# Griffan/VerifyBamID

Hardware: AMD Instinct MI355X
Metric: llk_evals_per_sec (higher is better)
Workload: dtype f64; 1 GPU; synthetic pileup 100000 markers x depth 30, --NumPC 4 (BASELINE.json configs[2] shape); parallelism=1 GPU, rccl_world_size=1, launched_by=single process, reads=2999230, active_markers=100000, distinct_codes=42, device=gfx950:sramecc+:xnack-

## Files before the change

### verifybamid_amd/csrc/kernel_debug.h

```cpp
#ifndef VB2_KERNEL_DEBUG_H_
#define VB2_KERNEL_DEBUG_H_

#ifndef VB2_ABLATE
#define VB2_ABLATE 0
#endif
#ifndef VB2_FLAG_RELEASE
#define VB2_FLAG_RELEASE 1
#endif
#ifndef VB2_SOFT_PROLOGUE
#define VB2_SOFT_PROLOGUE 1
#endif
#ifndef VB2_CTRL_PRIO
#define VB2_CTRL_PRIO 3
#endif
#ifndef VB2_STAMP_ROUND
#define VB2_STAMP_ROUND 0
#endif

namespace vb2 {
constexpr int kAblNoMap = 1, kAblNoTable = 2, kAblNoItems = 4, kAblNoReads = 8, kAblNoEpi = 16, kAblNoSignal = 32, kAblNoMul = 64, kAblNoRowLoads = 128;
constexpr int kAblate = VB2_ABLATE;
}

#ifdef VB2_WITH_STAMPS
#define VB2_STAMPS_OF(L) ((L).stamps)
#else
#define VB2_STAMPS_OF(L) (static_cast<unsigned long long*>(nullptr))
#endif

#ifdef VB2_ITEM_PROF
#define VB2_IP_T(var) const unsigned long long var = __builtin_readcyclecounter()
#define VB2_IP_USE(x) asm volatile("" ::"v"(x))
#else
#define VB2_IP_T(var)
#define VB2_IP_USE(x)
#endif

#endif
```

### verifybamid_amd/csrc/llk_kernels.hip

```cpp
#include "llk_kernels.h"

#include <hip/hip_runtime.h>
#include <link.h>

#include "kernel_debug.h"
#include "tile_sched.h"
#include "tunables.h"
#ifndef VB2_SIMD_DEAL
#define VB2_SIMD_DEAL 1
#endif

#include <algorithm>
#include <atomic>
#include <cstring>
#include <type_traits>
#include <vector>

namespace vb2 {

__device__ __forceinline__ void pair_of(int p, int& g1, int& g2)
{
    g1 = p >> 1;
    const int lo = p & 1;
    g2 = lo + (lo >= g1 ? 1 : 0);
// ... 212 lines not shown
    const double val = (alpha * e1 + one_minus_alpha * e2) * p_err +
                       (alpha * n1 + one_minus_alpha * n2) * p_ok;
    return log_tab(val, ltab_addr);
}

__device__ __forceinline__ double prob_entry(double alpha, double p_err, int g1, int g2)
{
    const double p_ok = 1.0 - p_err;
    const double e1 = (double)g1 * (1.0 / 6.0), e2 = (double)g2 * (1.0 / 6.0);
    const double n1 = 1.0 - 0.5 * (double)g1, n2 = 1.0 - 0.5 * (double)g2;
    const double one_minus_alpha = 1.0 - alpha;
    double val = (alpha * e1 + one_minus_alpha * e2) * p_err +
                 (alpha * n1 + one_minus_alpha * n2) * p_ok;
    return val >= 0.0 ? val : __builtin_nan("");
}

__device__ __forceinline__ void initial_gf(double af, double* gf)
{
    af = vmin_f64(vmax_f64(af, 0.00005), 0.99995);
    gf[0] = (1 - af) * (1 - af);
    gf[1] = 2 * (af) * (1 - af);
    gf[2] = af * af;
}


constexpr int kExpTabDoubles = 64 * 32;
constexpr int kPrefetch = 8;
constexpr int kPrefetchL2 = 2;

__device__ __forceinline__ void lane_map(int lane, int& m, int& g)
{
    const int q = (lane >> 2) & 7;
    const int nib = (0x76452310u >> (4 * q)) & 7;
    g = (nib & 1) + 2 * (lane >> 5);
    m = ((nib >> 1) << 2) + (lane & 3);
}
__device__ __forceinline__ int lane_of(int m, int g)
{
    const int idx = ((g & 1) << 2) + (m >> 2);
    const int q = (0x74216530u >> (4 * idx)) & 7;
    return ((g >> 1) << 5) + (q << 2) + (m & 3);
}

__device__ __forceinline__ int lane_xchg_i32(int x, int off, int partner)
{
    if (off == 1) return __builtin_amdgcn_update_dpp(0, x, 0xB1, 0xf, 0xf, true);
    if (off == 2) return __builtin_amdgcn_update_dpp(0, x, 0x4E, 0xf, 0xf, true);
    if (off == 4) {
        const int a = __builtin_amdgcn_update_dpp(0, x, 0x124, 0xf, 0x5, false);
        return __builtin_amdgcn_update_dpp(a, x, 0x12C, 0xf, 0xa, false);
    }
    return __shfl(x, partner, 64);
}
__device__ __forceinline__ double lane_xchg_f64(double x, int off, int partner)
{
    if (off == 1 || off == 2 || off == 4)
        return __hiloint2double(lane_xchg_i32(__double2hiint(x), off, partner), lane_xchg_i32(__double2loint(x), off, partner));
    return __shfl(x, partner, 64);
}

template <int MODE> struct Geom { static constexpr int kMaxWaves = 16, kBlocksPerCU = 1, kWavesPerSimd = 4; };
template <int MODE> struct ModeNp { static constexpr int value = MODE == 2 ? 8 : MODE == 4 ? 1 : MODE == 5 ? 2 : 4; };

struct InlinePoints {
    int count;
    double v[kInlinePointDoubles];
};

struct NoHook {
    __device__ bool on_block() const { return false; }
    __device__ bool mine() const { return false; }
    __device__ void run() {}
    __device__ bool keep_etab() const { return false; }
    __device__ bool prim_in_lds() const { return false; }
    __device__ bool keep_prim() const { return false; }
    __device__ double* sum_stage() const { return nullptr; }
    __device__ uint32_t cache_rec() const { return 0u; }
    __device__ unsigned int* sync_word() const { return nullptr; }
    __device__ bool collect_only() const { return false; }
    __device__ bool no_collect() const { return false; }
};
__host__ __device__ __forceinline__ bool eval_is_dynamic(const DeviceLayout& L, uint32_t nblk, int nwave, int ngrp)
{
    const uint32_t max_tiles_blk = owned_most(L.pd ? 1 : 0, (uint32_t)L.num_mt, nblk);
    return max_tiles_blk * (uint32_t)ngrp <= (uint32_t)(L.dyn_limit * nwave);
}

template <int MODE, bool W16 = false, class Hook = NoHook, bool STREAM = false, int QUEUE = -1, int KSEL = 0,
          bool LCACHE = false, int ESH = 8, bool PD = false, int SPLIT = 0>
__device__ __forceinline__ void
eval_body(const DeviceLayout& L, const double* ip_v, const int ip_count, const double* __restrict__ points, int num_valid,
          double* __restrict__ partials, double* __restrict__ llk_out,
          unsigned int* __restrict__ ticket, unsigned long long* __restrict__ done_flag,
          unsigned long long done_seq, const uint32_t blk, const uint32_t nblk,
          unsigned int* __restrict__ batch_done, unsigned int batch_active, const int ngrp_in,
          const unsigned long long tag, const Schedule sch, const bool coherent_points = false,
          const int tid_in = -1, const double* lds_rows = nullptr ,
          Hook hook = Hook())
{
    extern __shared__ __attribute__((aligned(16))) double lds[];
    static_assert(MODE >= 2 && MODE <= 5, "wave shapes 2..5");
    static_assert(!PD || ESH == 8, "probability-domain contexts have no exp table");
    static_assert(!(PD && W16) || ((MODE == 4 || MODE == 5) && STREAM), "8-bit step lists: cohort steps of one and two points");
    static_assert(!SPLIT || (PD && MODE == 2 && QUEUE == 1 && !STREAM && !LCACHE), "split launches: the 8-point shape on the queue");
    constexpr int OSH = PD ? 1 : 0;
    constexpr bool ONEGRP = MODE != 2 || STREAM;
    constexpr int KAF = KSEL > 0 ? 0 : -1;
    constexpr int BTL = MODE == 4 ? 1 : 2;
    constexpr int TPW = MODE == 3 ? 2 : (MODE == 4 || MODE == 5) ? 4 : 1;
    constexpr int SLOTS = 4 / TPW;
    constexpr int NP = SLOTS * BTL;
    const int row_bytes = MODE == 2 ? kRowBytesWide : L.row_bytes;
    const int RS = row_bytes >> 3;
    const int nrow = L.num_code + 1;
    const int nthread = blockDim.x;
    const int nwave = nthread >> 6;
    const int k = KSEL > 0 ? KSEL : L.num_pc;
    const int stride = 2 * k + 1;
    constexpr int NVS = SPLIT ? SPLIT : 1;
    const int g_per = SPLIT ? (ngrp_in + NVS - 1) / NVS : ngrp_in;
    const int g_lo = SPLIT ? (int)(blk % (uint32_t)NVS) * g_per : 0;
    const int ngrp = ONEGRP ? 1 : SPLIT ? (ngrp_in - g_lo < g_per ? ngrp_in - g_lo : g_per) : ngrp_in;
    const int p_off = g_lo * NP;
    const uint32_t vstep = SPLIT ? nblk / (uint32_t)NVS : 0u, vb0 = SPLIT ? blk / (uint32_t)NVS : blk;
    const double* const known_af_p = KAF == 0 ? nullptr : L.known_af;
    const int NPT = NP * ngrp;
    constexpr int kEtabCopies = (1 << ESH) / 8, kEtabDoubles = PD ? 0 : 64 * kEtabCopies;
    constexpr int kLtabDoubles = PD ? 0 : kLogTabDoubles;
    double* etab = lds;
    double* ltab = lds + kEtabDoubles;
    double* tab = ltab + kLtabDoubles;
    double* red = tab + ngrp * nrow * RS;
    unsigned int* queue = reinterpret_cast<unsigned int*>(red + NVS * NPT);
    double* pts = red + NVS * NPT + 2;
    double* ptq = pts + (size_t)NPT * stride + ((NPT * stride) & 1);
    const size_t prim_off = (size_t)(ptq - lds) + (size_t)NPT * 2 * k;
    double2* prim_lds = reinterpret_cast<double2*>(lds + prim_off + (prim_off & 1));
    double* tile_llk = reinterpret_cast<double*>(prim_lds + L.num_prim);

    const int tid = tid_in >= 0 ? tid_in : (int)threadIdx.x;
    const int lane = tid & 63;
    const int wave = __builtin_amdgcn_readfirstlane(tid >> 6);
    int m, g4;
    lane_map(lane, m, g4);
    const int g = g4 & (SLOTS - 1);
    const int half = TPW == 1 ? 0 : g4 / SLOTS;
    const bool stamp_this = VB2_STAMP_ROUND == 0 || (unsigned)(tag & 0xffffffffull) == (unsigned)VB2_STAMP_ROUND;
#ifdef VB2_ITEM_PROF
    unsigned long long* stamps = nullptr;
#else
    unsigned long long* stamps = (VB2_STAMPS_OF(L) && stamp_this) ? VB2_STAMPS_OF(L) + (size_t)blk * 8 : nullptr;
#endif
    if (stamps && tid == 0) { stamps[0] = wall_clock64(); stamps[4] = 0; }

    const bool collect_only = hook.collect_only();
    if (collect_only && hook.mine()) hook.run();
    if (!collect_only) {
    const bool hook_blk = hook.on_block(), hook_mine = hook.mine();
    unsigned int* const soft_word = PD ? hook.sync_word() : nullptr;
    const bool soft = hook_blk && soft_word != nullptr;
    if (soft && hook_mine) hook.run();
    const int ptid = !soft ? tid : hook_mine ? 0x3fffffff : tid - 64, pnthread = soft ? nthread - 64 : nthread;
    unsigned int soft_gen = 0;
    auto prologue_sync = [&]() {
        if (!soft) { __syncthreads(); return; }
        if (hook_mine) return;
        soft_gen += (unsigned int)(nwave - 1);
        if (lane == 0) __hip_atomic_fetch_add(soft_word, 1u, __ATOMIC_RELAXED, __HIP_MEMORY_SCOPE_WORKGROUP);
        while (__hip_atomic_load(soft_word, __ATOMIC_RELAXED, __HIP_MEMORY_SCOPE_WORKGROUP) < soft_gen) __builtin_amdgcn_s_sleep(1);
        asm volatile("" ::: "memory");
    };
    if (ptid == 0) *queue = (unsigned int)(nwave - (hook_blk ? 1 : 0));
    for (int e = ptid; e < NPT * stride; e += pnthread) {
        const int b = e / stride;
        const int src = p_off + b < num_valid ? p_off + b : num_valid - 1;
        const int idx = src * stride + (e - b * stride);
        const double v = (kAblate & kAblNoMap) ? 0.01 * (double)(1 + idx % 7)
                         : lds_rows ? lds_rows[idx]
                         : ip_count > 0 ? ip_v[idx]
                         : coherent_points ? __hip_atomic_load(&points[idx], __ATOMIC_RELAXED, __HIP_MEMORY_SCOPE_AGENT)
                                           : points[idx];
        pts[e] = v;
        const int c = e - b * stride;
        if (c < 2 * k) ptq[((b / BTL) * 2 * k + c) * BTL + (b % BTL)] = v;
    }
    if (!PD && !hook.keep_etab() && tid < kLogTabDoubles / 2)
        reinterpret_cast<double2*>(ltab)[tid] = kLogTabRows[tid];
    if (!PD && !hook.keep_etab())
        for (int jb = 2 * wave; jb < 64; jb += 2 * nwave) {
            const double t0 = kExp2Tab[jb], t1 = kExp2Tab[jb + 1];
            const double tv = lane < 32 ? exp_tab_entry(t0, jb) : exp_tab_entry(t1, jb + 1);
            if constexpr (ESH == 8) etab[jb * 32 + lane] = tv;
            else if ((lane & 31) < kEtabCopies) etab[(jb + (lane >> 5)) * kEtabCopies + (lane & 31)] = tv;
        }
    const bool prim_kept = hook.prim_in_lds() && hook.keep_prim();
    const bool staged = ngrp > 1 || (hook.prim_in_lds() && !prim_kept) || (PD && L.num_pair > 0 && !prim_kept);
    if (staged)
        for (int e = ptid; e < L.num_prim; e += pnthread) prim_lds[e] = L.prim[e];
    const bool early_table = lds_rows != nullptr && !staged;
    if (!early_table) prologue_sync();
    if (stamps && (soft ? ptid : tid) == 0) stamps[1] = wall_clock64();

    const uint32_t ltab_addr = lds_byte_addr(ltab);
    const int num_single = PD ? L.num_prim - L.num_pair : L.num_prim;
    for (int e = ptid; e < ((kAblate & kAblNoTable) ? 0 : num_single * 6 * NP); e += pnthread) {
        const int pi = e / (6 * NP);
        const int bp = e - pi * (6 * NP);
        const int bb = bp / 6, p = bp - bb * 6;
        const double2 rec = (staged || prim_kept) ? prim_lds[pi] : L.prim[pi];
        const uint32_t pr = (uint32_t)__double_as_longlong(rec.y);
        const int dc = (int)(pr & 0xffffu), twin = (int)(pr >> 16);
        int g1, g2;
        pair_of(p, g1, g2);
        if constexpr (PD && !ONEGRP) {
            constexpr int kSide = 3;
            for (int g0 = 0; g0 < ngrp; g0 += kSide) {
                double v3[kSide], r3[kSide];
                double* cell3[kSide];
#pragma unroll
                for (int u = 0; u < kSide; ++u) {
                    const int ge = g0 + u < ngrp ? g0 + u : ngrp - 1;
                    v3[u] = prob_entry(pts[(ge * NP + bb) * stride + 2 * k], rec.x, g1, g2);
                    r3[u] = v3[u];
                    cell3[u] = tab + (size_t)ge * nrow * RS + dc * RS + bp;
                    *cell3[u] = r3[u];
                }
                const int kq = twin & 0xff, pstride = RS * (int)(int8_t)(twin >> 8);
                for (int n = 1; n < kq; ++n) {
#pragma unroll
                    for (int u = 0; u < kSide; ++u) {
                        r3[u] *= v3[u];
                        cell3[u] += pstride;
                        *cell3[u] = r3[u];
                    }
                }
            }
        } else
#pragma clang loop unroll(disable)
        for (int grp_e = 0; grp_e < ngrp; ++grp_e) {
            const double alpha_e = early_table ? lds_rows[(bb < num_valid ? bb : num_valid - 1) * stride + 2 * k]
                                               : pts[(grp_e * NP + bb) * stride + 2 * k];
            double* gtab = tab + (size_t)grp_e * nrow * RS;
            if constexpr (PD) {
                const double v = prob_entry(alpha_e, rec.x, g1, g2);
                double r = v;
                double* cell = gtab + dc * RS + bp;
                constexpr int kMir = kPdAltOffset / 8;
                const int mir = kMir + bb * 6 + (5 - p) - bp;
                *cell = r;
                if constexpr (NP <= 4 && STREAM) cell[mir] = r;
                const int kq = twin & 0xff, pstride = RS * (int)(int8_t)(twin >> 8);
                for (int n = 1; n < kq; ++n) {
                    r *= v;
                    cell += pstride;
                    *cell = r;
                    if constexpr (NP <= 4 && STREAM) cell[mir] = r;
                }
            } else {
                const double v = table_entry(alpha_e, rec.x, g1, g2, ltab_addr);
                const double tv = W16 ? 0.5 * v : v;
                gtab[dc * RS + bp] = tv;
                if (twin != 0xffff) gtab[twin * RS + bb * 6 + (5 - p)] = tv;
            }
        }
    }
    for (int e = ptid; e < ngrp * RS; e += pnthread) {
        const int grp_e = e / RS;
        tab[((size_t)grp_e * nrow + L.num_code) * RS + (e - grp_e * RS)] = PD ? 1.0 : 0.0;
    }
    if constexpr (PD) {
        for (int level = 0; level < 2 && L.num_pair > 0 && !(kAblate & kAblNoTable); ++level) {
            const int nrec = level == 0 ? L.num_pair - L.num_pair2 : L.num_pair2;
            if (nrec == 0) break;
            prologue_sync();
            const double2* const prec = prim_lds + num_single + (level == 0 ? 0 : L.num_pair - L.num_pair2);
            for (int e = ptid; e < nrec * 6 * NP; e += pnthread) {
                const int pi = e / (6 * NP);
                const int bp = e - pi * (6 * NP);
                const double2 rec = prec[pi];
                const uint32_t ab = (uint32_t)__double_as_longlong(rec.x), dst = (uint32_t)__double_as_longlong(rec.y);
                const int ra = (int)(ab & 0xffffu) * RS + bp, rb = (int)(ab >> 16) * RS + bp, rd = (int)dst * RS + bp;
                constexpr int kMir = kPdAltOffset / 8;
                const int bb = bp / 6, p = bp - bb * 6;
                const int mir = kMir + bb * 6 + (5 - p) - bp;
#pragma clang loop unroll(disable)
                for (int grp_e = 0; grp_e < ngrp; ++grp_e) {
                    double* gtab = tab + (size_t)grp_e * nrow * RS;
                    const double v = gtab[ra] * gtab[rb];
                    gtab[rd] = v;
                    if constexpr (NP <= 4 && STREAM) gtab[rd + mir] = v;
                }
            }
        }
    }
    prologue_sync();
    if (stamps && (soft ? ptid : tid) == 0) stamps[2] = wall_clock64();

    const uint32_t nt_v0 = owned_count(OSH, (uint32_t)L.num_mt, vb0, nblk);
    const uint32_t nt_v1 = SPLIT ? owned_count(OSH, (uint32_t)L.num_mt, vb0 + vstep, nblk) : 0u;
    const uint32_t nt_v2 = SPLIT > 2 ? owned_count(OSH, (uint32_t)L.num_mt, vb0 + 2u * vstep, nblk) : 0u;
    auto nt_of = [&](uint32_t vs) { return vs == 0u ? nt_v0 : vs == 1u ? nt_v1 : nt_v2; };
    const uint32_t ntile_blk = nt_v0;
    const size_t mp = L.m_pad;
    const uint32_t nunit = SPLIT ? (uint32_t)NVS * ntile_blk : (ntile_blk + TPW - 1) / TPW;
    const uint32_t nitem = (kAblate & kAblNoItems) ? 0u : nunit * (uint32_t)ngrp;
    const float inv_nunit = 1.0f / (float)(nunit ? nunit : 1u);
    const uint32_t ngrp_magic = ngrp > 1 ? 0xFFFFFFFFu / (uint32_t)ngrp + 1u : 0u;
    const bool dyn = QUEUE < 0 ? eval_is_dynamic(L, nblk, nwave, ngrp) : QUEUE != 0;
    typedef unsigned int __attribute__((ext_vector_type(2))) vuint2;
    typedef __attribute__((address_space(1))) const vuint2 g_cuint2;
    typedef __attribute__((address_space(1))) const double g_cdouble;
    typedef __attribute__((address_space(1))) const char g_cchar;
    g_cuint2* const g_rec = (g_cuint2*)(W16 ? L.mt_rec16 : L.mt_rec);
    g_cuint2* const g_codes = (g_cuint2*)(W16 ? L.codes16 : L.codes);
    typedef __attribute__((address_space(1))) const uint32_t g_cuint;
    typedef __attribute__((address_space(3))) const uint32_t lds_cuint;
    typedef typename std::conditional<PD, uint32_t, vuint2>::type RowWord;
    constexpr uint32_t kRowBytes = PD ? kMtMarkers * 4u : kMtMarkers * 8u, kLaneBytes = PD ? 4u : 8u;
    g_cdouble* const g_ediag = (g_cdouble*)L.ediag;
    g_cdouble* const g_ud = (g_cdouble*)L.ud;
    g_cdouble* const g_mu = (g_cdouble*)L.mu;
    g_cdouble* const g_kaf = (g_cdouble*)known_af_p;
    auto tile_product = [&](ScaledProd* p, bool cross) {
#pragma unroll
        for (int off = 8; off >= 1; off >>= 1) {
            const int partner = lane_of(m ^ off, g4);
#pragma unroll
            for (int t = 0; t < BTL; ++t) {
                p[t].m *= lane_xchg_f64(p[t].m, off, partner);
                p[t].e += lane_xchg_f64(p[t].e, off, partner);
            }
        }
        if (!cross) return;
#pragma unroll
        for (int off = SLOTS; off < 4; off <<= 1) {
            const int partner = lane_of(m, g4 ^ off);
#pragma unroll
            for (int t = 0; t < BTL; ++t) {
                p[t].m *= __shfl(p[t].m, partner, 64);
                p[t].e += __shfl(p[t].e, partner, 64);
            }
        }
    };
    LaneProd wave_prod[BTL];
#pragma unroll
    for (int t = 0; t < BTL; ++t) wave_prod[t] = LaneProd{1.0, 0};
    int nfactor = 0;
    auto renorm_wave = [&]() {
#pragma unroll
        for (int t = 0; t < BTL; ++t) {
            wave_prod[t].e += __builtin_amdgcn_frexp_exp(wave_prod[t].m);
            wave_prod[t].m = __builtin_amdgcn_frexp_mant(wave_prod[t].m);
        }
        nfactor = 0;
    };
    uint32_t grp_wave = 0;
    auto flush_wave = [&](uint32_t grp) {
// ... 445 lines not shown
                if (r < end && (r & 1)) row_step(kS1, alt_tag, alt_tag, kNotFirst);
                while (r + 1 < end) {
                    row_step(kS0, alt_tag, alt_tag, kNotFirst);
                    row_step(kS1, alt_tag, alt_tag, kNotFirst);
                }
                if (r < end) row_step(kS0, alt_tag, alt_tag, kNotFirst);
            };
            rows_of_kind(rows_ra, kRef);
            if ((steps_ref & 1) && r == rows_ra && r < rows) {
                if (r & 1) row_step(kS1, kRef, kAltT, kNotFirst);
                else row_step(kS0, kRef, kAltT, kNotFirst);
            }
            rows_of_kind(rows, kAltT);
            if constexpr (PIPE) {
                issue_rows(rec_n2, have_next);
                cst_nx = other_const(mt_next, have_next);
                rec_nx = rec_n2;
            }
        } else if constexpr (PIPE) {
            const bool more = __any(rows > kPf);
            walk_block(0, more, std::false_type());
            if (more)
                for (int s0 = kPf; s0 < rows; s0 += kPf) walk_block(s0, true, std::false_type());
            issue_rows(rec_n2, have_next);
            cst_nx = other_const(mt_next, have_next);
            rec_nx = rec_n2;
        } else if constexpr (PEEL) {
            if (rows > 0) {
                walk_block(0, true, std::true_type());
                for (int s0 = kPf; s0 < rows; s0 += kPf) walk_block(s0, true, std::false_type());
            } else {
#pragma unroll
                for (int i = 0; i < BTL * 6; ++i) acc[i] = cst;
            }
        } else {
            for (int s0 = 0; s0 < rows; s0 += kPf) walk_block(s0, true, std::false_type());
        }

        __builtin_amdgcn_s_setprio(0);
#ifdef VB2_STAMP_CTRL
        if (stamps && lane == 0 && wave == 1 && !hook_blk) stamps[3] = wall_clock64();
#else
        if (stamps && lane == 0 && wave == 1) stamps[3] = wall_clock64();
#endif
        VB2_IP_USE(acc[0]); VB2_IP_USE(acc[BTL * 6 - 1]);
        VB2_IP_T(ip_t3);
        VB2_IP_USE(e0); VB2_IP_USE(e1); VB2_IP_USE(e2); VB2_IP_USE(mur); VB2_IP_USE(udr[0]); VB2_IP_USE(udr[3]);
        VB2_IP_T(ip_t4);
        double lk_m[BTL];
        int lk_e[BTL];
        marker_lk(live, pos, acc, e0, e1, e2, udr, mur, my_ptq, lk_m, lk_e, cst);
        VB2_IP_USE(lk_m[0]); VB2_IP_USE(lk_m[BTL - 1]);
        VB2_IP_T(ip_t5);
        if (!dyn) {
#pragma unroll
            for (int t = 0; t < BTL; ++t) {
                wave_prod[t].m *= lk_m[t];
                wave_prod[t].e += lk_e[t];
            }
            if (++nfactor == kLazyRenorm) renorm_wave();
            if (have_sched) {
                ++s_i;
                idx = PIPE ? idx_next : (s_i < s_end ? (uint32_t)sch.item[s_i] : nitem);
                continue;
            }
            ++round;
            idx = round * (uint32_t)nwave + ((round & 1u) ? (uint32_t)(nwave - 1 - wave) : (uint32_t)wave);
            continue;
        }
#pragma unroll
        for (int off = 8; off >= 1; off >>= 1) {
            const int partner = lane_of(m ^ off, g4);
#pragma unroll
            for (int t = 0; t < BTL; ++t) {
                lk_m[t] *= lane_xchg_f64(lk_m[t], off, partner);
                lk_e[t] += lane_xchg_i32(lk_e[t], off, partner);
            }
        }
        if (m == 0 && have_tile) {
#pragma unroll
            for (int t = 0; t < BTL; ++t) {
                const size_t o = ((((size_t)grp * NVS + vs) * ntile_blk + it) * NP + g * BTL + t) * 2;
                tile_llk[o] = lk_m[t];
                tile_llk[o + 1] = (double)lk_e[t];
            }
        }
        VB2_IP_T(ip_t6);
        idx = draw_item();
#ifdef VB2_ITEM_PROF
        {
            const unsigned long long ip_t7 = __builtin_readcyclecounter();
            ip_sum[0] += ip_t1 - ip_t0; ip_sum[1] += ip_t2 - ip_t1; ip_sum[2] += ip_t3 - ip_t2; ip_sum[3] += ip_t4 - ip_t3;
            ip_sum[4] += ip_t5 - ip_t4; ip_sum[5] += ip_t6 - ip_t5; ip_sum[6] += ip_t7 - ip_t6; ip_sum[7] += 1;
        }
#endif
    }
#ifdef VB2_ITEM_PROF
    if (VB2_STAMPS_OF(L) && lane == 0 && dyn)
        for (int i = 0; i < 8; ++i) atomicAdd(&VB2_STAMPS_OF(L)[(size_t)blk * 8 + i], ip_sum[i]);
#endif
    if (!dyn) {
        for (uint32_t grp = grp_wave; grp < (uint32_t)ngrp; ++grp) flush_wave(grp);
    }

    if (stamps && lane == 0 && !hook_mine) atomicMax(&stamps[4], wall_clock64());
    const uint32_t nres = dyn ? ntile_blk : (uint32_t)nwave;
    __syncthreads();
    {
        const uint32_t j16 = (uint32_t)lane & 15u;
        for (int b = tid >> 4; b < NVS * NPT; b += nthread >> 4) {
            const int vsb = SPLIT ? b / NPT : 0, bl = b - vsb * NPT;
            const int grp = bl / NP, bb = bl - grp * NP;
            ScaledProd p{1.0, 0.0};
            const uint32_t nres_b = SPLIT ? nt_of((uint32_t)vsb) : nres;
            for (uint32_t i = j16; i < nres_b; i += 16) {
                const size_t o = ((((size_t)grp * NVS + vsb) * nres + i) * NP + bb) * 2;
                p.m *= tile_llk[o];
                p.e += tile_llk[o + 1];
                sp_renorm(p);
            }
            auto row_move = [&](double x, auto ctrl) -> double {
                constexpr int kCtrl = decltype(ctrl)::value;
                return __hiloint2double(__builtin_amdgcn_update_dpp(0, __double2hiint(x), kCtrl, 0xf, 0xf, false),
                                        __builtin_amdgcn_update_dpp(0, __double2loint(x), kCtrl, 0xf, 0xf, false));
            };
            auto row_step = [&](auto ctrl) {
                const double om = row_move(p.m, ctrl), oe = row_move(p.e, ctrl);
                p.m *= om;
                p.e += oe;
            };
            row_step(std::integral_constant<int, 0x140>());
            row_step(std::integral_constant<int, 0x141>());
            row_step(std::integral_constant<int, 0xB1>());
            row_step(std::integral_constant<int, 0x4E>());
            sp_renorm(p);
            if (j16 == 0) red[b] = log_nonneg(p.m) + p.e * 6.93147180559945286227e-01;
        }
    }
    __syncthreads();
    if (VB2_STAMPS_OF(L) && tid == 0) {
        const unsigned long long t5 = wall_clock64();
        if (stamps) stamps[5] = t5;
        if (blk == 0 && nblk > 32 && !hook.no_collect()) VB2_STAMPS_OF(L)[20 * 8 + 7] += t5 - VB2_STAMPS_OF(L)[7];
    }
    }
    auto put_result = [&](int b, double v) {
        if (done_flag) __hip_atomic_store(&llk_out[b], v, __ATOMIC_RELAXED, __HIP_MEMORY_SCOPE_SYSTEM);
        else llk_out[b] = v;
    };
    if (ticket == nullptr) {
        if (tid < NPT) partials[(size_t)tid * nblk + blk] = red[tid];
        return;
    }
    if (tag == 0) {
        if (tid < NVS * NPT) {
            const int vsb = SPLIT ? tid / NPT : 0, bl = tid - vsb * NPT;
            __hip_atomic_store(&partials[(size_t)(p_off + bl) * nblk + (vb0 + (uint32_t)vsb * vstep)], red[tid],
                               __ATOMIC_RELAXED, __HIP_MEMORY_SCOPE_AGENT);
        }
        asm volatile("s_waitcnt vmcnt(0)" ::: "memory");
        __syncthreads();
        unsigned int* last_flag = queue;
        if (tid == 0) {
            const unsigned int t = __hip_atomic_fetch_add(ticket, 1u, __ATOMIC_RELAXED,
                                                          __HIP_MEMORY_SCOPE_AGENT);
            *last_flag = (t == nblk - 1) ? 1u : 0u;
        }
        __syncthreads();
        if (*last_flag == 0u) return;
        const int nbt = (int)nblk;
        constexpr int kSide = 3;
        for (int b0 = wave; b0 < num_valid; b0 += kSide * nwave) {
            double s[kSide];
#pragma unroll
            for (int u = 0; u < kSide; ++u) s[u] = 0;
            for (int base = 0; base < nbt; base += 8 * 64) {
                double x[kSide][8];
#pragma unroll
                for (int u = 0; u < kSide; ++u) {
                    const int b = b0 + u * nwave;
                    const double* p = partials + (size_t)(b < num_valid ? b : b0) * nbt;
#pragma unroll
                    for (int q = 0; q < 8; ++q) {
                        const int i = base + q * 64 + lane;
                        x[u][q] = i < nbt ? __hip_atomic_load(&p[i], __ATOMIC_RELAXED, __HIP_MEMORY_SCOPE_AGENT)
                                          : 0.0;
                    }
                }
#pragma unroll
                for (int u = 0; u < kSide; ++u)
#pragma unroll
                    for (int q = 0; q < 8; ++q) s[u] += x[u][q];
            }
#pragma unroll
            for (int u = 0; u < kSide; ++u) {
                const int b = b0 + u * nwave;
                const double t = wave_sum(s[u]);
                if (lane == 0 && b < num_valid) put_result(b, t);
            }
        }
        if (tid == 0) __hip_atomic_store(ticket, 0u, __ATOMIC_RELAXED, __HIP_MEMORY_SCOPE_AGENT);
    } else {
    unsigned long long* pw = reinterpret_cast<unsigned long long*>(partials);
    if (wave == 0 && !collect_only) {
        const unsigned long long bits = lane < NPT ? (unsigned long long)__double_as_longlong(red[lane]) : 0ull;
        if (lane < NPT)
            __hip_atomic_store(&pw[(size_t)lane * nblk + blk], bits, __ATOMIC_RELAXED, __HIP_MEMORY_SCOPE_AGENT);
        unsigned long long x = lane < NPT ? word_hash(bits, (unsigned)lane) : 0ull;
        int top = 1;
        while (top < NPT) top <<= 1;
        for (int off = top >> 1; off >= 1; off >>= 1) x ^= __shfl_xor(x, off, 64);
        if (lane == 0)
            __hip_atomic_store(&pw[(size_t)NPT * nblk + blk], x ^ resident_mix(tag), __ATOMIC_RELAXED,
                               __HIP_MEMORY_SCOPE_AGENT);
    }
    if (collect_only ? false : (blk != 0 || hook.no_collect())) return;
    if (!hook.sum_stage()) __syncthreads();
    const int nb = (int)nblk;
    double* stage = hook.sum_stage() ? hook.sum_stage() : lds;
    {
        const unsigned long long want = resident_mix(tag);
        const unsigned long long t_wait = wall_clock64();
        for (int b = tid; b < nb; b += nthread) {
            for (unsigned it = 0;; ++it) {
                unsigned long long x = __hip_atomic_load(&pw[(size_t)NPT * nb + b], __ATOMIC_RELAXED,
                                                         __HIP_MEMORY_SCOPE_AGENT);
                for (int w0 = 0; w0 < NPT; w0 += NP) {
                    unsigned long long v[NP];
#pragma unroll
                    for (int u = 0; u < NP; ++u)
                        v[u] = __hip_atomic_load(&pw[(size_t)(w0 + u) * nb + b], __ATOMIC_RELAXED,
                                                 __HIP_MEMORY_SCOPE_AGENT);
#pragma unroll
                    for (int u = 0; u < NP; ++u) {
                        x ^= word_hash(v[u], (unsigned)(w0 + u));
                        stage[(size_t)(w0 + u) * nb + b] = __longlong_as_double((long long)v[u]);
                    }
                }
                if (x == want) break;
                if ((it & 63) == 63 && wall_clock64() - t_wait > kHandoffGiveUpTicks) {
                    for (int w = 0; w < NPT; ++w) stage[(size_t)w * nb + b] = __builtin_nan("");
                    break;
                }
                __builtin_amdgcn_s_sleep(1);
            }
        }
    }
    __syncthreads();
    for (int b = wave; b < num_valid; b += nwave) {
        const double* p = stage + (size_t)b * nb;
        double s = 0;
        for (int base = 0; base < nb; base += 8 * 64) {
            double x[8];
#pragma unroll
            for (int q = 0; q < 8; ++q) {
                const int i = base + q * 64 + lane;
                x[q] = i < nb ? p[i] : 0.0;
            }
#pragma unroll
            for (int q = 0; q < 8; ++q) s += x[q];
        }
        s = wave_sum(s);
        if (lane == 0) put_result(b, s);
    }
    }
    if (VB2_STAMPS_OF(L) && tid == 0) {
        const unsigned long long t6 = wall_clock64();
        if (stamps) stamps[6] = t6;
        if ((collect_only || (blk == 0 && !hook.no_collect())) && nblk > 32) VB2_STAMPS_OF(L)[21 * 8 + 7] += t6 - VB2_STAMPS_OF(L)[7];
    }
    if (done_flag && !(kAblate & kAblNoSignal)) {
        asm volatile("s_waitcnt vmcnt(0)" ::: "memory");
        __syncthreads();
        if (tid == 0) {
            bool signal = true;
            if (batch_done) {
                const unsigned int t = __hip_atomic_fetch_add(batch_done, 1u, __ATOMIC_RELAXED, __HIP_MEMORY_SCOPE_AGENT);
                signal = (t == batch_active - 1);
                if (signal) __hip_atomic_store(batch_done, 0u, __ATOMIC_RELAXED, __HIP_MEMORY_SCOPE_AGENT);
            }
            if (signal)
                __hip_atomic_store(done_flag, done_seq, VB2_FLAG_RELEASE ? __ATOMIC_RELEASE : __ATOMIC_RELAXED, __HIP_MEMORY_SCOPE_SYSTEM);
        }
    }
}

template <int MODE, int QUEUE, int KSEL = 0, bool PD = false>
__global__ void __launch_bounds__(Geom<MODE>::kMaxWaves * 64, Geom<MODE>::kWavesPerSimd)
llk_eval_kernel(const DeviceLayout L, const InlinePoints ip, const double* __restrict__ points,
                int num_valid, double* __restrict__ partials, double* __restrict__ llk_out,
                unsigned int* __restrict__ ticket, unsigned long long* __restrict__ done_flag,
                unsigned long long done_seq, int ngrp, unsigned long long tag, const Schedule sch)
{
    eval_body<MODE, false, NoHook, false, QUEUE, KSEL, false, 8, PD>(L, ip.v, ip.count, points, num_valid, partials, llk_out, ticket,
                                                                     done_flag, done_seq, blockIdx.x, gridDim.x, nullptr, 0u, ngrp, tag, sch);
}

template <int KSEL, int S>
__global__ void __launch_bounds__(Geom<2>::kMaxWaves * 64, Geom<2>::kWavesPerSimd)
llk_eval_split_kernel(const DeviceLayout L, const double* __restrict__ points, int num_valid, double* __restrict__ partials,
                      double* __restrict__ llk_out, unsigned int* __restrict__ ticket, unsigned long long* __restrict__ done_flag,
                      unsigned long long done_seq, int ngrp)
{
    eval_body<2, false, NoHook, false, 1, KSEL, false, 8, true, S>(L, nullptr, 0, points, num_valid, partials, llk_out, ticket, done_flag,
                                                                     done_seq, blockIdx.x, gridDim.x, nullptr, 0u, ngrp, 0ull,
                                                                     Schedule{nullptr, nullptr});
}

template <int KSEL, bool PD = false>
__global__ void __launch_bounds__(Geom<2>::kMaxWaves * 64, Geom<2>::kWavesPerSimd)
llk_eval_passes_kernel(const DeviceLayout L, const double* __restrict__ points, int num_valid, int points_per_pass,
                       double* __restrict__ partials, double* __restrict__ llk_out, unsigned int* __restrict__ tickets,
                       unsigned long long* __restrict__ done_flag, unsigned long long done_seq,
                       unsigned long long* __restrict__ scratch_flag)
{
    const int stride = 2 * L.num_pc + 1;
    int pass = 0;
    for (int first = 0; first < num_valid; first += points_per_pass, ++pass) {
        const int left = num_valid - first;
        const int nv = left < points_per_pass ? left : points_per_pass;
        const bool last = left <= points_per_pass;
        if (pass > 0) __syncthreads();
        eval_body<2, false, NoHook, false, 1, KSEL, false, (PD ? 8 : 6), PD>(
            L, nullptr, 0, points + (size_t)first * stride, nv, partials + (size_t)first * gridDim.x, llk_out + first,
            tickets + pass, (last || !done_flag) ? done_flag : scratch_flag, done_seq, blockIdx.x, gridDim.x, nullptr, 0u,
            (nv + 7) / 8, 0ull, Schedule{nullptr, nullptr});
    }
}

#define VB2_PASSES_KERNEL_ARGS                                                                                           \
    const DeviceLayout, const double*, int, int, double*, double*, unsigned int*, unsigned long long*, unsigned long long, \
        unsigned long long*
#if defined(VB2_TU_MAIN)
extern template __global__ void llk_eval_passes_kernel<4>(VB2_PASSES_KERNEL_ARGS);
extern template __global__ void llk_eval_passes_kernel<2>(VB2_PASSES_KERNEL_ARGS);
extern template __global__ void llk_eval_passes_kernel<0>(VB2_PASSES_KERNEL_ARGS);
extern template __global__ void llk_eval_passes_kernel<4, true>(VB2_PASSES_KERNEL_ARGS);
extern template __global__ void llk_eval_passes_kernel<2, true>(VB2_PASSES_KERNEL_ARGS);
extern template __global__ void llk_eval_passes_kernel<0, true>(VB2_PASSES_KERNEL_ARGS);
#elif defined(VB2_TU_PASSES)
template __global__ void llk_eval_passes_kernel<4>(VB2_PASSES_KERNEL_ARGS);
template __global__ void llk_eval_passes_kernel<2>(VB2_PASSES_KERNEL_ARGS);
template __global__ void llk_eval_passes_kernel<0>(VB2_PASSES_KERNEL_ARGS);
template __global__ void llk_eval_passes_kernel<4, true>(VB2_PASSES_KERNEL_ARGS);
template __global__ void llk_eval_passes_kernel<2, true>(VB2_PASSES_KERNEL_ARGS);
template __global__ void llk_eval_passes_kernel<0, true>(VB2_PASSES_KERNEL_ARGS);
#endif

template <int MODE, bool W16, int KSEL = 0, int STATIC = 0, bool PD = false>
__global__ void __launch_bounds__(Geom<MODE>::kMaxWaves * 64, Geom<MODE>::kWavesPerSimd)
llk_eval_multi_kernel(const DeviceLayout* __restrict__ layouts, const Schedule* __restrict__ scheds,
                      const double* __restrict__ points,
                      const int* __restrict__ num_valid, double* __restrict__ partials,
                      double* __restrict__ llk_out, unsigned int* __restrict__ tickets, int bps,
// ... 605 lines not shown
```

Measured before the change: 1.018 million evals/s.

## Split ticket reduction per point-class and prefetch table inputs before prologue sync

For SPLIT kernels, table-building inputs (prim records and allele values) are now loaded from global memory with a one-step software prefetch, and the prologue barrier is skipped so table construction overlaps the point staging. The final cross-block reduction uses one ticket counter per split class, so each class's last block reduces only its own points, and wave 0 alone signals when the partials fit in one wave. It also records the XCC id in debug stamps. This adds risk: skipping the prologue sync could race with LDS data that later code expects to be staged, and the per-class ticket logic assumes nblk is divisible by NVS.

```diff
diff --git a/verifybamid_amd/csrc/kernel_debug.h b/verifybamid_amd/csrc/kernel_debug.h
--- a/verifybamid_amd/csrc/kernel_debug.h
+++ b/verifybamid_amd/csrc/kernel_debug.h
@@ -13,6 +13,9 @@
 #ifndef VB2_CTRL_PRIO
 #define VB2_CTRL_PRIO 3
 #endif
+#ifndef VB2_SPLIT_FAST
+#define VB2_SPLIT_FAST 3
+#endif
 #ifndef VB2_STAMP_ROUND
 #define VB2_STAMP_ROUND 0
 #endif
@@ -20,6 +23,7 @@
 namespace vb2 {
 constexpr int kAblNoMap = 1, kAblNoTable = 2, kAblNoItems = 4, kAblNoReads = 8, kAblNoEpi = 16, kAblNoSignal = 32, kAblNoMul = 64, kAblNoRowLoads = 128;
 constexpr int kAblate = VB2_ABLATE;
+constexpr int kSplitFast = VB2_SPLIT_FAST;
 }
 
 #ifdef VB2_WITH_STAMPS
diff --git a/verifybamid_amd/csrc/llk_kernels.hip b/verifybamid_amd/csrc/llk_kernels.hip
--- a/verifybamid_amd/csrc/llk_kernels.hip
+++ b/verifybamid_amd/csrc/llk_kernels.hip
@@ -388,6 +388,13 @@
     unsigned long long* stamps = (VB2_STAMPS_OF(L) && stamp_this) ? VB2_STAMPS_OF(L) + (size_t)blk * 8 : nullptr;
 #endif
     if (stamps && tid == 0) { stamps[0] = wall_clock64(); stamps[4] = 0; }
+    if constexpr (SPLIT != 0) {
+        if (stamps && tid == 0 && blk != 0u && blk != 20u && blk != 21u) {
+            unsigned int xcc;
+            asm volatile("s_getreg_b32 %0, hwreg(HW_REG_XCC_ID)" : "=s"(xcc));
+            stamps[7] = 1ull + (xcc & 15u);
+        }
+    }
 
     const bool collect_only = hook.collect_only();
     if (collect_only && hook.mine()) hook.run();
@@ -406,6 +413,25 @@
         while (__hip_atomic_load(soft_word, __ATOMIC_RELAXED, __HIP_MEMORY_SCOPE_WORKGROUP) < soft_gen) __builtin_amdgcn_s_sleep(1);
         asm volatile("" ::: "memory");
     };
+    constexpr bool SPLIT_EARLY = SPLIT != 0 && (kSplitFast & 1) != 0;
+    constexpr int kTabSide = 3;
+    const int ntab_split = (kAblate & kAblNoTable) ? 0 : (PD ? L.num_prim - L.num_pair : L.num_prim) * 6 * NP;
+    auto table_inputs = [&](int e, int g0, double2& rec_o, double* al_o) {
+        const int pi = e / (6 * NP);
+        const int bb = (e - pi * (6 * NP)) / 6;
+        rec_o = L.prim[pi];
+#pragma unroll
+        for (int u = 0; u < kTabSide; ++u) {
+            const int ge = g0 + u < ngrp ? g0 + u : ngrp - 1;
+            const int b = ge * NP + bb;
+            const int idx = (p_off + b < num_valid ? p_off + b : num_valid - 1) * stride + 2 * k;
+            al_o[u] = (kAblate & kAblNoMap) ? 0.01 * (double)(1 + idx % 7) : points[idx];
+        }
+    };
+    double2 tin_rec = make_double2(0.0, 0.0);
+    double tin_al[kTabSide] = {0.0, 0.0, 0.0};
+    if constexpr (SPLIT_EARLY)
+        if (ptid < ntab_split) table_inputs(ptid, 0, tin_rec, tin_al);
     if (ptid == 0) *queue = (unsigned int)(nwave - (hook_blk ? 1 : 0));
     for (int e = ptid; e < NPT * stride; e += pnthread) {
         const int b = e / stride;
@@ -434,11 +460,56 @@
     if (staged)
         for (int e = ptid; e < L.num_prim; e += pnthread) prim_lds[e] = L.prim[e];
     const bool early_table = lds_rows != nullptr && !staged;
-    if (!early_table) prologue_sync();
+    if (!early_table && !SPLIT_EARLY) prologue_sync();
     if (stamps && (soft ? ptid : tid) == 0) stamps[1] = wall_clock64();
 
     const uint32_t ltab_addr = lds_byte_addr(ltab);
     const int num_single = PD ? L.num_prim - L.num_pair : L.num_prim;
+    if constexpr (SPLIT_EARLY) {
+        int e = ptid, g0 = 0;
+        while (e < ntab_split) {
+            int e_n = e, g0_n = g0 + kTabSide;
+            if (g0_n >= ngrp) {
+                g0_n = 0;
+                e_n = e + pnthread;
+            }
+            double2 rec_n = tin_rec;
+            double al_n[kTabSide] = {tin_al[0], tin_al[1], tin_al[2]};
+            if (e_n < ntab_split) table_inputs(e_n, g0_n, rec_n, al_n);
+            const int pi = e / (6 * NP);
+            const int bp = e - pi * (6 * NP);
+            const int bb = bp / 6, p = bp - bb * 6;
+            (void)bb;
+            const uint32_t pr = (uint32_t)__double_as_longlong(tin_rec.y);
+            const int dc = (int)(pr & 0xffffu), twin = (int)(pr >> 16);
+            int g1, g2;
+            pair_of(p, g1, g2);
+            double v3[kTabSide], r3[kTabSide];
+            double* cell3[kTabSide];
+#pragma unroll
+            for (int u = 0; u < kTabSide; ++u) {
+                const int ge = g0 + u < ngrp ? g0 + u : ngrp - 1;
+                v3[u] = prob_entry(tin_al[u], tin_rec.x, g1, g2);
+                r3[u] = v3[u];
+                cell3[u] = tab + (size_t)ge * nrow * RS + dc * RS + bp;
+                *cell3[u] = r3[u];
+            }
+            const int kq = twin & 0xff, pstride = RS * (int)(int8_t)(twin >> 8);
+            for (int n = 1; n < kq; ++n) {
+#pragma unroll
+                for (int u = 0; u < kTabSide; ++u) {
+                    r3[u] *= v3[u];
+                    cell3[u] += pstride;
+                    *cell3[u] = r3[u];
+                }
+            }
+            tin_rec = rec_n;
+#pragma unroll
+            for (int u = 0; u < kTabSide; ++u) tin_al[u] = al_n[u];
+            e = e_n;
+            g0 = g0_n;
+        }
+    } else
     for (int e = ptid; e < ((kAblate & kAblNoTable) ? 0 : num_single * 6 * NP); e += pnthread) {
         const int pi = e / (6 * NP);
         const int bp = e - pi * (6 * NP);
@@ -1190,25 +1261,52 @@
         if (tid < NPT) partials[(size_t)tid * nblk + blk] = red[tid];
         return;
     }
+    constexpr bool SPLIT_CLASS = SPLIT != 0 && (kSplitFast & 2) != 0;
+    unsigned int* const my_ticket = SPLIT_CLASS && ticket ? ticket + blk % (uint32_t)NVS : ticket;
+    if constexpr (SPLIT_CLASS) {
+        batch_done = ticket ? ticket + NVS : nullptr;
+        batch_active = (unsigned int)NVS;
+    }
     if (tag == 0) {
         if (tid < NVS * NPT) {
             const int vsb = SPLIT ? tid / NPT : 0, bl = tid - vsb * NPT;
             __hip_atomic_store(&partials[(size_t)(p_off + bl) * nblk + (vb0 + (uint32_t)vsb * vstep)], red[tid],
                                __ATOMIC_RELAXED, __HIP_MEMORY_SCOPE_AGENT);
         }
+        unsigned int* last_flag = queue;
+        if constexpr (SPLIT_CLASS) {
+            if (NVS * NPT <= 64) {
+                if (wave == 0) {
+                    asm volatile("s_waitcnt vmcnt(0)" ::: "memory");
+                    if (lane == 0) {
+                        const unsigned int t = __hip_atomic_fetch_add(my_ticket, 1u, __ATOMIC_RELAXED, __HIP_MEMORY_SCOPE_AGENT);
+                        *last_flag = (t == nblk / (uint32_t)NVS - 1) ? 1u : 0u;
+                    }
+                }
+            } else {
+                asm volatile("s_waitcnt vmcnt(0)" ::: "memory");
+                __syncthreads();
+                if (tid == 0) {
+                    const unsigned int t = __hip_atomic_fetch_add(my_ticket, 1u, __ATOMIC_RELAXED, __HIP_MEMORY_SCOPE_AGENT);
+                    *last_flag = (t == nblk / (uint32_t)NVS - 1) ? 1u : 0u;
+                }
+            }
+        } else {
         asm volatile("s_waitcnt vmcnt(0)" ::: "memory");
         __syncthreads();
-        unsigned int* last_flag = queue;
         if (tid == 0) {
             const unsigned int t = __hip_atomic_fetch_add(ticket, 1u, __ATOMIC_RELAXED,
                                                           __HIP_MEMORY_SCOPE_AGENT);
             *last_flag = (t == nblk - 1) ? 1u : 0u;
         }
+        }
         __syncthreads();
         if (*last_flag == 0u) return;
         const int nbt = (int)nblk;
-        constexpr int kSide = 3;
-        for (int b0 = wave; b0 < num_valid; b0 += kSide * nwave) {
+        constexpr int kSide = SPLIT_CLASS ? 1 : 3;
+        const int pt_lo = SPLIT_CLASS ? p_off : 0;
+        const int pt_hi = SPLIT_CLASS ? (p_off + NPT < num_valid ? p_off + NPT : num_valid) : num_valid;
+        for (int b0 = pt_lo + wave; b0 < pt_hi; b0 += kSide * nwave) {
             double s[kSide];
 #pragma unroll
             for (int u = 0; u < kSide; ++u) s[u] = 0;
@@ -1217,7 +1315,7 @@
 #pragma unroll
                 for (int u = 0; u < kSide; ++u) {
                     const int b = b0 + u * nwave;
-                    const double* p = partials + (size_t)(b < num_valid ? b : b0) * nbt;
+                    const double* p = partials + (size_t)(b < pt_hi ? b : b0) * nbt;
 #pragma unroll
                     for (int q = 0; q < 8; ++q) {
                         const int i = base + q * 64 + lane;
@@ -1234,10 +1332,10 @@
             for (int u = 0; u < kSide; ++u) {
                 const int b = b0 + u * nwave;
                 const double t = wave_sum(s[u]);
-                if (lane == 0 && b < num_valid) put_result(b, t);
-            }
-        }
-        if (tid == 0) __hip_atomic_store(ticket, 0u, __ATOMIC_RELAXED, __HIP_MEMORY_SCOPE_AGENT);
+                if (lane == 0 && b < pt_hi) put_result(b, t);
+            }
+        }
+        if (tid == 0) __hip_atomic_store(my_ticket, 0u, __ATOMIC_RELAXED, __HIP_MEMORY_SCOPE_AGENT);
     } else {
     unsigned long long* pw = reinterpret_cast<unsigned long long*>(partials);
     if (wave == 0 && !collect_only) {
```

Result: faster. 1.053 million evals/s, median of 6 (+3.5%).
